# nilspin/VoxelHashing_demo

Hardware: AMD Instinct MI355X
Metric: frames/s TSDF-integrated + raycast Mpix/s, 640×480, 1/2/4/8 MI355X (higher is better)
Workload: dtype f32

## Files before the change

voxelhashing_demo_amd/csrc/vh_api_model.hip:

```cpp

static int sweep_and_release(vh_context *c)
{
    int rc;
    if (c->fp.flags & kFlagOverflow) {
        rc = launch(c, kPhaseGc, gc_sweep_overflow_a_kernel, dim3(256), dim3(256), c->fp, c->dp);
        if (rc == VH_OK) rc = launch(c, kPhaseGc, gc_sweep_overflow_b_kernel, dim3(256), dim3(256), c->fp, c->dp);
    } else {
        rc = launch(c, kPhaseGc, gc_sweep_kernel, dim3(256), dim3(256), c->fp, c->dp);
    }
    if (rc != VH_OK) return rc;
    rc = release_color(c);
    if (rc != VH_OK) return rc;
    rc = launch(c, kPhaseGc, gc_release_kernel, dim3(1024), dim3(256), c->dp);
    if (rc != VH_OK) return rc;
    rc = launch(c, kPhaseGc, gc_finish_kernel, dim3(1), dim3(1), c->dp, c->occupiedCounter);
    if (rc != VH_OK) return rc;
    if (c->profiling) c->times.gc_calls += 1;
    c->params.numOccupiedBlocks = 0;
    VH_HIP(hipGetLastError());
    return VH_OK;
}

extern "C" int vh_delete_blocks(vh_context *c, const int32_t *d_keys, int32_t n)
{
// ... 333 lines not shown
                   : fail(VH_ERR_HIP, "snapshot upload failed; the model was reset to empty", e);
    }
    std::memcpy(c->params.global_transform, h.params.global_transform, sizeof c->fp.T);
    std::memcpy(c->params.inv_global_transform, h.params.inv_global_transform, sizeof c->fp.Tinv);
    std::memcpy(c->fp.T, h.params.global_transform, sizeof c->fp.T);
    std::memcpy(c->fp.Tinv, h.params.inv_global_transform, sizeof c->fp.Tinv);
    std::memcpy(c->fp.proj, h.proj, sizeof h.proj);
    c->params.numOccupiedBlocks = 0;
    c->epochTotal = h.epoch;
    return VH_OK;
}

extern "C" int vh_set_option(vh_context *c, const char *name, int value)
{
    if (c) { DeviceGuard fguard(c->device); const int frc = flush_pending(c); if (frc != VH_OK) return frc; }
    if (!c || !name) return fail(VH_ERR_INVALID_ARGUMENT, "null argument");
    if (std::strcmp(name, "flatten_variant") == 0) {
        if (value != kWalkStridedBallot && value != kWalkIndexed)
            return fail(VH_ERR_INVALID_ARGUMENT, "flatten_variant: 3 (the reference's walk) or 4 (occupancy index)");
        c->flattenVariant = value;
        return VH_OK;
    }
    if (std::strcmp(name, "walk_nt") == 0) {
        c->fp.flags = value ? (c->fp.flags | kFlagWalkNt) : (c->fp.flags & ~kFlagWalkNt);
        return VH_OK;
    }
    if (std::strcmp(name, "walk_reverse") == 0) { c->walkReverse = value != 0; return VH_OK; }
    if (std::strcmp(name, "walk_short") == 0) {
        c->fp.flags = value ? (c->fp.flags | kFlagWalkShort) : (c->fp.flags & ~kFlagWalkShort);
        return VH_OK;
    }
    if (std::strcmp(name, "claim_lead") == 0 && value >= -1) { c->claimLead = value; return VH_OK; }
#ifdef VH_DEBUG_SKIP_ROLES
    if (std::strcmp(name, "debug_skip_roles") == 0 && value >= 0 && value < 32) {
        c->debugSkipRoles = value;
        if (value & 16) c->fp.flags |= kFlagDebugNoProbe; else c->fp.flags &= ~kFlagDebugNoProbe;
        return VH_OK;
    }
#endif
    if (std::strcmp(name, "spin_limit") == 0 && value >= 0) { c->spinLimit = (uint32_t)value; return VH_OK; }
    if (std::strcmp(name, "pipeline_overflow") == 0 && value >= 0 && value <= 2) {
        DeviceGuard g(c->device);
        const int frc = flush_pending(c);
        if (frc != VH_OK) return frc;
        c->pipelineOverflow = value;
        return VH_OK;
    }
    if (std::strcmp(name, "gen_frames_per_launch") == 0 && value >= 1 && value <= kGenBatch) { c->genFramesPerLaunch = value; return VH_OK; }
    if (std::strcmp(name, "pipeline_shards") == 0) {
        if (value < 0 || value > 2) return fail(VH_ERR_INVALID_ARGUMENT, "pipeline_shards: 0, 1 or 2");
        if (value < 2) { DeviceGuard g(c->device); const int frc = flush_pending(c, PendingFrame::kMulti); if (frc != VH_OK) return frc; }
        c->pipelineShards = value;
        return VH_OK;
    }
    if (std::strcmp(name, "pipeline") == 0) {
        c->pipeline = value != 0;
        return VH_OK;
    }
    if (std::strcmp(name, "overflow_list") == 0) {
        if (c->epochTotal != 0 && ((c->fp.flags & kFlagOverflow) != 0u) != (value != 0))
            return fail(VH_ERR_INVALID_ARGUMENT, "overflow_list must be chosen before the first frame");
        if (c->fp.listSize < 2 && value) return fail(VH_ERR_INVALID_ARGUMENT, "attachedLinkedListSize must be at least 2");
        c->fp.flags = value ? (c->fp.flags | kFlagOverflow) : (c->fp.flags & ~kFlagOverflow);
        return VH_OK;
    }
    if (std::strcmp(name, "band_mode") == 0 && (value == VH_BAND_RAY || value == VH_BAND_NORMAL_DDA || value == VH_BAND_RAY_DDA)) {
        c->fp.flags &= ~(kFlagBandDda | kFlagBandRayDda);
// ... 124 lines not shown
```

voxelhashing_demo_amd/csrc/vh_api_shard.hip:

```cpp

static void make_view_frustum(const vh_context *c, const float pose[16], float t_min, float t_max, float f[22])
{
    float inv[16];
    invert4x4(pose, inv);
    std::memcpy(f, inv, 12 * sizeof(float));
    const float r = 7.0f * c->fp.voxelSize;
    const float a[4] = {(0.0f - c->rc_cx) / c->rc_fx, ((float)(c->fp.width - 1) - c->rc_cx) / c->rc_fx,
                        (0.0f - c->rc_cy) / c->rc_fy, ((float)(c->fp.height - 1) - c->rc_cy) / c->rc_fy};
    for (int i = 0; i < 4; ++i) {
        f[12 + i] = a[i];
        f[16 + i] = -(r * sqrtf(1.0f + a[i] * a[i]));
    }
    f[20] = t_min - r;
    f[21] = t_max + r;
}

extern "C" int vh_export_views(vh_context *c, const float *poses, int32_t n_views, float t_min, float t_max,
                               vh_view_record *d_records, int32_t capacity, int32_t *d_counts)
{
    if (!c || !poses || !d_records || !d_counts) return fail(VH_ERR_INVALID_ARGUMENT, "null argument");
    if (n_views < 1 || n_views > VH_MAX_CAMERAS) return fail(VH_ERR_INVALID_ARGUMENT, "1..VH_MAX_CAMERAS views");
    if (capacity < 1) return fail(VH_ERR_INVALID_ARGUMENT, "capacity must be positive");
    if (!(t_max > t_min)) return fail(VH_ERR_INVALID_ARGUMENT, "t_max must exceed t_min");
    if (c->viewBlocks) return fail(VH_ERR_INVALID_ARGUMENT, "a view table has no voxels of its own to export");
// ... 302 lines not shown
        for (int j = 0; j < n; ++j) {
            const int rc = vh_set_pose(c, poses + 16 * (size_t)(b0 + j));
            if (rc != VH_OK) return rc;
            if (!d_depth[b0 + j]) return fail(VH_ERR_INVALID_ARGUMENT, "null depth image");
            std::memcpy(fr.T[j], c->fp.T, sizeof fr.T[j]);
            std::memcpy(fr.Tinv[j], c->fp.Tinv, sizeof fr.Tinv[j]);
            fr.depth[j] = d_depth[b0 + j];
        }
        write_packets_u16_kernel<<<dim3(64, (unsigned)n), 256, 0, c->stream>>>(
            fr, (int32_t)npix, d_packets + packet_frame_stride * (size_t)b0, packet_frame_stride);
    }
    VH_HIP(hipGetLastError());
    return VH_OK;
}

struct MultiBatch {
    const int4 *bins;
    const float *packets;
    int32_t numBins, capacity, binStride, frameStride, numCams;
    size_t packetStride, packetFrameStride;
    bool perBatch;
};

static int launch_multi_pipelined(vh_context *c, const MultiBatch *mb, int b, const GenJob *job)
{
    PendingFrame &pend = c->pend;
    const bool doNew = mb != nullptr, hasOld = pend.kind == PendingFrame::kMulti;
    if (!doNew && !hasOld) return VH_OK;
    int rc;
    if (doNew && (rc = vh_reset_mutexes(c)) != VH_OK) return rc;
    uint32_t *maskOf[2] = {c->dp.compactMask, c->maskBuf2};
    MultiPipeArgs a;
    std::memset(&a, 0, sizeof a);
    PipeRotation r = pipe_rotation(c, a, a, doNew, hasOld);
    a.numEntries = (uint32_t)c->numEntries;
    a.numCams = doNew ? mb->numCams : pend.numCams;
    a.packetStride = doNew ? mb->packetStride : pend.packetStride;
    if (doNew) {
        a.partsPerBin = bin_parts(mb->capacity); a.numBins = (uint32_t)mb->numBins;
        a.claimBlocks = a.numBins * a.partsPerBin;
        a.walkShort = multi_walk_short(c) ? 1u : 0u;
        a.walkIndexed = multi_walk_indexed(c) ? 1u : 0u;
        a.walkBlocks = multi_walk_blocks(c);
        a.capacity = mb->capacity; a.binStride = mb->binStride;
        a.binsNew = mb->bins + (size_t)mb->frameStride * b;
        a.binFrame = mb->perBatch ? b : -1;
        a.packetsNew = mb->packets + mb->packetFrameStride * b;
    }
    a.commitBlocks = hasOld ? (uint32_t)c->commitBlocks : 0u;
    a.integrateBlocks = hasOld ? (uint32_t)c->pipeIntegrateGrid : 0u;
    a.claimSpan = claim_span(c, a.claimBlocks, a.walkBlocks);
    a.claimRatio = claim_ratio(a.claimBlocks, a.claimSpan);
    a.epochOld = pend.epoch;
    a.packetsOld = pend.packets;
    r.dpNew.compactMask = maskOf[r.newParity];
    a.claimOld = r.dpOld.claim; a.candOld = r.dpOld.candidates; a.compactOld = r.dpOld.compact; a.maskOld = maskOf[r.oldParity];
    a.candCapacityOld = r.dpOld.candCapacity;
    const bool sensor = (doNew ? c->packetFormat : pend.packetFormat) == VH_PACKET_U16;
    const bool serial = (c->fp.flags & kFlagOverflow) != 0u;
    const bool gen = job && job->blocks && doNew && sensor && !serial;
    if (gen) a.gen = *job;
    const dim3 grid(a.commitBlocks + a.integrateBlocks + (gen ? a.gen.blocks : 0u) + a.claimBlocks + a.walkBlocks);
    using Yes = std::true_type;
    using No = std::false_type;
    auto go = [&](auto sensorC, auto serialC, auto indexedC, auto genC) {
        return launch(c, kPhaseFramePipelined,
                      frame_multi_pipelined_kernel<decltype(sensorC)::value, decltype(serialC)::value, decltype(indexedC)::value, decltype(genC)::value>,
                      grid, dim3(256), c->fp, r.dpNew, a);
    };
    if (gen) rc = with_bool(a.walkIndexed != 0u, [&](auto i) { return go(Yes{}, No{}, i, Yes{}); });
    else if (a.walkIndexed) rc = with_bool(sensor, [&](auto s) { return go(s, No{}, Yes{}, No{}); });
    else rc = with_bool(sensor, [&](auto s) { return with_bool(serial, [&](auto q) { return go(s, q, No{}, No{}); }); });
    if (rc != VH_OK) return rc;
    pipe_launched(c, r, serial, doNew ? PendingFrame::kMulti : PendingFrame::kNone, hasOld, false, hasOld);
    if (doNew) {
        pend.epoch = c->fp.epoch;
        pend.packets = a.packetsNew;
        pend.packetStride = mb->packetStride;
        pend.numCams = mb->numCams;
        pend.packetFormat = c->packetFormat;
    }
    return VH_OK;
}

static bool multi_can_pipeline(const vh_context *c, int32_t num_bins, int32_t capacity)
{
    return can_pipeline(c, (uint32_t)num_bins * bin_parts(capacity) + (uint32_t)grid_for(c->numEntries, kFlattenThreads * kEntriesPerLaneShort));
}

static bool multi_can_fuse_generation(const vh_context *c, int32_t num_bins, int32_t capacity)
{
    return c->pipelineShards && multi_can_pipeline(c, num_bins, capacity) && !(c->fp.flags & kFlagOverflow) &&
           c->packetFormat == VH_PACKET_U16 && !(c->fp.allocBand > 0.0f) && c->flattenVariant != kWalkIndexed;
}

static bool multi_fusing_pays(const vh_context *c)
{
    return (size_t)c->numEntries * sizeof(VoxelEntry) > ((size_t)60 << 20);
}

static int vh_apply_frames_batch_gen(vh_context *c, int32_t batch, const int32_t *d_bins, int32_t num_bins,
                                     int32_t capacity, int32_t bin_stride, int32_t frame_stride, int32_t num_cams,
                                     const float *d_packets, size_t packet_stride, size_t packet_frame_stride, const GenJob *jobs);

// ... 140 lines not shown
```

voxelhashing_demo_amd/csrc/vh_frame.hip:

```cpp
#pragma once

namespace vh {

__device__ __forceinline__ bool grouped_role(uint32_t r, uint32_t claimBlocks, uint32_t claimSpan, uint32_t claimRatio,
                                             uint32_t claimLead, uint32_t &index)
{
    const uint32_t g = (r >> 3) - claimLead, q = r & 7u;
    uint32_t before = (int32_t)g < 0 ? 0u : (claimBlocks + 7u) >> 3;
    if (g < claimSpan) {
        const unsigned long long phase = (unsigned long long)q << 29;
        before = (uint32_t)(((unsigned long long)g * claimRatio + phase) >> 32);
        const uint32_t after = (uint32_t)(((unsigned long long)(g + 1u) * claimRatio + phase) >> 32);
        if (after != before) { index = 8u * before + q; return true; }
    }
    index = r - 8u * before;
    return false;
}

template <int kKind, class In>
__global__ __launch_bounds__(256) void frame_scan_claim_kernel(const FrameParams fp, const DevPtrs dp, const In in,
                                                               uint32_t numEntries, uint32_t claimBlocks,
                                                               int parity, float *__restrict__ planeOut, uint32_t claimSpan,
                                                               uint32_t claimRatio, uint32_t walkGroups, uint32_t walkReverse,
                                                               uint32_t claimLead)
// ... 146 lines not shown
    kLeanIndexedWaveNt = 8,
    kLeanBuilds = 9
};
struct LeanBuild { uint32_t flags; bool indexed, claimPerWave; };
constexpr LeanBuild lean_build(int kLean)
{
    return {kFlagWalkShort | (kLean % 2 == 0 ? kFlagWalkNt : 0u) | (kLean == kLeanRayDda || kLean == kLeanRayDdaNt ? kFlagBandRayDda : 0u),
            kLean >= kLeanIndexed, kLean >= kLeanIndexedWave};
}

template <bool kSerial>
__device__ __forceinline__ bool pending_live(uint32_t hasOld, const int32_t *counters, int32_t setOld)
{
    if (kSerial) return hasOld != 0u;
    return hasOld && counters[kPipeHeapFree + setOld] >= counters[kPipeWinners + setOld];
}

template <class In, class Depth>
struct PipeKernargs {
    FrameParams fpNew;
    DevPtrs dpNew;
    In inNew;
    FrameParams fpOld;
    DevPtrs dpOld;
    Depth depthOld;
    PipeArgs a;
};
template <class In, class Depth>
struct PipeSignature {
    PipeLeadWords lead;
    PipeKernargs<In, Depth> rest;
};

template <class In, class Depth, int kLean>
__device__ __forceinline__ const PipeKernargs<In, Depth> &role_arguments()
{
    typedef PipeKernargs<In, Depth> K;
    typedef PipeSignature<In, Depth> Signature;
    static_assert(offsetof(Signature, lead) == 0 && offsetof(Signature, rest) == sizeof(PipeLeadWords),
                  "frame_pipelined_kernel(lead, rest): rest lies right behind lead");
    typedef const __attribute__((address_space(4))) char *SegmentBytes;
    typedef const __attribute__((address_space(4))) K *SegmentPtr;
    SegmentPtr p = (SegmentPtr)((SegmentBytes)__builtin_amdgcn_kernarg_segment_ptr() + offsetof(Signature, rest));
    asm volatile("" : "+s"(p));
    const K &k = *(const K *)p;
    constexpr uint32_t leanFlags = lean_build(kLean).flags;
    if (kLean != kLeanNone) {
        __builtin_assume(k.fpNew.flags == leanFlags);
        __builtin_assume(k.fpOld.flags == leanFlags);
    }
    return k;
}

template <class In, class Depth, bool kBand, bool kSerial, int kLean>
__device__ __forceinline__ void frame_pipelined(const PipeLead &l)
{
    typedef PipeKernargs<In, Depth> K;
    constexpr LeanBuild lean = lean_build(kLean);
    const bool walkIndexed = kLean != kLeanNone ? lean.indexed : l.walkIndexed != 0u;
    constexpr bool serial = kSerial;
    const uint32_t b = blockIdx.x;
    uint32_t role, index;
    if (b < l.commitBlocks) { role = 0; index = b; }
    else if (walkIndexed) {
        const uint32_t r = b - l.commitBlocks;
        if (r < l.walkBlocks) { role = 3; index = r; }
        else if (r < l.walkBlocks + l.integrateBlocks) { role = 1; index = r - l.walkBlocks; }
        else { role = 2; index = r - l.walkBlocks - l.integrateBlocks; }
    }
    else if (b < l.commitBlocks + l.integrateBlocks) { role = 1; index = b - l.commitBlocks; }
    else {
        const bool claims = grouped_role(b - l.commitBlocks - l.integrateBlocks, l.claimBlocks, l.claimSpan, l.claimRatio, l.claimLead, index);
        role = claims ? 2u : 3u;
        if (claims && index >= l.claimBlocks) return;
    }
#ifdef VH_DEBUG_SKIP_ROLES
    if (l.skipRoles & (1u << role)) {
        const K &k = role_arguments<In, Depth, kLean>();
// ... 150 lines not shown
```

voxelhashing_demo_amd/csrc/vh_shard.hip:

```cpp
#pragma once

namespace vh {

constexpr int kBinFrameMarks = 0x40000000;

__device__ __forceinline__ void claim_bin_slice(const FrameParams &fp, const DevPtrs &dp,
                                                const int4 *__restrict__ bins, int32_t capacity, int32_t binStride,
                                                uint32_t binIndex, uint32_t part, uint32_t parts, int candCounter,
                                                const Pending &pend = kNoPending, int frame = -1)
{
    const int4 *bin = bins + (size_t)binIndex * binStride;
    const int4 head = bin[0];
    int n = head.x;
    const bool frameMarks = frame >= 0 && (head.w & kBinFrameMarks) != 0;
    const int room = frameMarks ? capacity - 3 : capacity - 1;
    int lo = 0, hiMark = 0;
    if (frameMarks) {
        const int4 c0 = bin[capacity - 2], c1 = bin[capacity - 1];
        const int cnt[8] = {c0.x, c0.y, c0.z, c0.w, c1.x, c1.y, c1.z, c1.w};
        n = 0;
#pragma unroll
        for (int f = 0; f < 8; ++f) {
            if (f == frame) lo = n;
            n += cnt[f];
            if (f == frame) hiMark = n;
        }
    }
    if (n > room) {
        if (part == 0 && threadIdx.x == 0) atomicAdd(dp.counters + kBinOverflow, 1);
        n = room;
    }
    if (frameMarks) {
        lo = min(lo, n);
        n = min(hiMark, n);
    } else if (frame >= 0 && head.w != 0) {
        const int per = head.w & 0xff, marks = (head.w >> 8) & 0xff, g = frame / per;
        const int m0 = min(head.y, n), m1 = min(head.z, n);
        lo = g == 0 ? 0 : g == 1 ? m0 : m1;
        n = g < marks ? (g == 0 ? m0 : m1) : n;
        if (g > 2) lo = n;
    }
#ifdef VH_DEBUG_SKIP_ROLES
    if (fp.flags & kFlagDebugNoProbe) n = min(n, lo + ((n - lo) >> 5));
#endif
    for (int i = lo + (int)part * 256 + (int)threadIdx.x; i < n; i += (int)parts * 256) {
        const int4 k = bin[1 + i];
        uint32_t rank = (uint32_t)k.w;
        if (frame >= 0) {
            if ((rank >> kRankCameraShift) != (uint32_t)frame) continue;
            rank = (binIndex << kRankCameraShift) | (rank & ((1u << kRankCameraShift) - 1u));
        }
        const uint32_t h = hash_block(k.x, k.y, k.z, fp.numBuckets);
        if (h < fp.bucketLo || h >= fp.bucketHi) continue;
        probe_and_claim(fp, dp, k.x, k.y, k.z, h, rank, candCounter, pend);
    }
}

__global__ __launch_bounds__(256) void claim_bins_kernel(const FrameParams fp, const DevPtrs dp,
                                                         const int4 *__restrict__ bins, int32_t capacity,
                                                         int32_t binStride)
{
    claim_bin_slice(fp, dp, bins, capacity, binStride, blockIdx.y, blockIdx.x, gridDim.x, kCandCount);
}

__device__ __forceinline__ uint32_t camera_mask(const FrameParams &fp, const int *pos, int32_t numCams,
                                                const float *__restrict__ packets, size_t packetStride)
{
    uint32_t seen = 0;
    for (int c = 0; c < numCams; ++c) {
        const float *pk = packets + packetStride * c;
        if (block_in_frustum(fp, pk, pk + 16, pos[0], pos[1], pos[2])) seen |= 1u << c;
    }
    return seen;
}

template <int kN = kEntriesPerLane>
__device__ __forceinline__ void flatten_multi_tile(const FrameParams &fp, const DevPtrs &dp, uint32_t numEntries,
                                                   uint32_t tileIndex, int32_t numCams,
                                                   const float *__restrict__ packets, size_t packetStride,
                                                   int counter, const Pending &pend = kNoPending)
{
    const uint32_t tile = tileIndex * (kFlattenThreads * kN);
    int32_t ptrs[kN];
    walk_load_tile(fp, dp, numEntries, tileIndex, ptrs);
    uint32_t seen[kN];
    int myCount = 0;
#pragma unroll
    for (int j = 0; j < kN; ++j) {
        seen[j] = 0;
        if (ptrs[j] == VH_FREE_BLOCK) continue;
        const uint32_t e = tile + j * kFlattenThreads + threadIdx.x;
        const VoxelEntry ent = dp.table[e];
        if (pend.claim && pend.live) {
            const uint32_t b = e / fp.bucketSize;
            const unsigned long long w = pend.claim[b];
            if (claim_epoch(w) == pend.epoch && claim_f(w) == e - b * fp.bucketSize) continue;
        }
        seen[j] = camera_mask(fp, ent.pos, numCams, packets, packetStride);
        myCount += seen[j] != 0u;
    }
    int slot = reserve_compact_slots(dp, counter, myCount);
    if (slot < 0) return;
#pragma unroll
    for (int j = 0; j < kN; ++j) {
        if (seen[j] == 0u) continue;
        dp.compact[slot] = dp.table[tile + j * kFlattenThreads + threadIdx.x];
        dp.compactMask[slot] = seen[j];
        ++slot;
    }
}

struct IndexSinkMulti {
    const FrameParams &fp;
    int32_t numCams;
    const float *__restrict__ packets;
    size_t packetStride;
    int counterIndex;
    __device__ __forceinline__ uint32_t judge(const VoxelEntry &e) const { return camera_mask(fp, e.pos, numCams, packets, packetStride); }
    __device__ __forceinline__ int counter() const { return counterIndex; }
    __device__ __forceinline__ void emit(const DevPtrs &dp, uint32_t pos, const VoxelEntry &e, uint32_t seen) const
    {
        dp.compact[pos] = e;
        dp.compactMask[pos] = seen;
    }
};

__global__ __launch_bounds__(kFlattenThreads) void flatten_multi_kernel(const FrameParams fp, const DevPtrs dp,
                                                                        uint32_t numEntries, int32_t numCams,
                                                                        const float *__restrict__ packets,
                                                                        size_t packetStride)
{
    flatten_multi_tile(fp, dp, numEntries, blockIdx.x, numCams, packets, packetStride, kCompactCount);
}

template <bool kSensor>
__device__ __forceinline__ auto packet_depth(const float *pk)
{
    if constexpr (kSensor) return DepthSensor{reinterpret_cast<const uint16_t *>(pk + kPacketHeaderU16), pk[32], pk[33], pk[34], pk[35]};
    else return DepthPlane{pk + kPacketHeader, 1};
}

template <bool kSensor>
// ... 79 lines not shown
                    dp.compactMask[slot] = seen;
                }
            }
        }
        __syncthreads();
        if (inserted && newMask != 0u)
            integrate_block_multi<kSensor>(fp, dp, newEntry, newMask, numCams, packets, packetStride);
        __syncthreads();
    }
    close_commit_fused(dp.counters, workers, parity, scanCount, 0, demanded);
}

#ifndef VH_FUSED_GEN_GROUPS
#define VH_FUSED_GEN_GROUPS 6
#endif
#ifndef VH_FUSED_GEN_PRIO
#define VH_FUSED_GEN_PRIO 3
#endif
constexpr int kFusedGenGroups = VH_FUSED_GEN_GROUPS;
struct GenJob {
    uint32_t blocks;
    int32_t numShards, capacity, binStride;
    int4 *bins;
    float *packet;
    const uint16_t *depth;
    uint32_t rankBase;
    float T[16], Tinv[16], k[9], unit;
    int4 *clearBins;
    int32_t clearStride;
    int32_t frame, batch;
};


struct MultiPipeArgs {
    uint32_t claimBlocks, walkBlocks, commitBlocks, integrateBlocks;
    uint32_t partsPerBin, numBins, numEntries;
    int32_t capacity, binStride, numCams;
    int32_t binFrame;
    int32_t doneTag;
    uint32_t spinLimit;
    int32_t setNew, setOld, setClear;
    uint32_t hasNew, hasOld;
    uint32_t walkShort;
    uint32_t walkIndexed;
    uint32_t claimSpan, claimRatio;
    uint32_t epochOld;
    const int4 *binsNew;
    const float *packetsNew, *packetsOld;
    size_t packetStride;
    unsigned long long *claimOld;
    int4 *candOld;
    VoxelEntry *compactOld;
    uint32_t *maskOld;
    uint32_t candCapacityOld;
    GenJob gen;
};

template <bool kSensor, bool kSerial, bool kIndexed = false, bool kGen = false>
__global__ __launch_bounds__(256) void frame_multi_pipelined_kernel(const FrameParams fp, const DevPtrs dp, const MultiPipeArgs a)
{
    if (!a.hasOld && blockIdx.x == 0u && threadIdx.x == 0) dp.counters[kPipeHeapFree + a.setNew] = dp.counters[kHeapCounter] + 1;
    if constexpr (kGen) {
        const uint32_t g0 = a.commitBlocks + a.integrateBlocks;
        if (blockIdx.x >= g0 && blockIdx.x < g0 + a.gen.blocks) {
            const uint32_t g = blockIdx.x - g0;
            if (VH_FUSED_GEN_PRIO) __builtin_amdgcn_s_setprio(VH_FUSED_GEN_PRIO);
            FrameParams fg = fp;
#pragma unroll
            for (int i = 0; i < 16; ++i) { fg.T[i] = a.gen.T[i]; fg.Tinv[i] = a.gen.Tinv[i]; }
            SensorImage in;
            in.depth = a.gen.depth;
#pragma unroll
            for (int i = 0; i < 9; ++i) in.k[i] = a.gen.k[i];
            in.unit = a.gen.unit;
            float *pk = a.gen.packet;
            if (g == 0 && threadIdx.x < kPacketHeaderU16) {
                const int t = threadIdx.x;
                pk[t] = t < 16 ? a.gen.T[t] : t < 32 ? a.gen.Tinv[t - 16] : t == 32 ? a.gen.k[6] : t == 33 ? a.gen.k[7] : t == 34 ? a.gen.k[8] : a.gen.unit;
            }
            if (g == 0 && a.gen.clearBins && (int)threadIdx.x < a.gen.numShards) {
                int4 *nb = a.gen.clearBins + (size_t)threadIdx.x * a.gen.clearStride;
                nb[0] = make_int4(0, 0, 0, kBinFrameMarks | a.gen.batch);
                nb[a.gen.capacity - 2] = make_int4(0, 0, 0, 0);
                nb[a.gen.capacity - 1] = make_int4(0, 0, 0, 0);
            }
#pragma unroll
            for (int j = 0; j < kFusedGenGroups; ++j) {
                const int idx = ((int)g * kFusedGenGroups + j) * 256 + (int)threadIdx.x;
                if (idx < fp.width * fp.height) reinterpret_cast<uint16_t *>(pk + kPacketHeaderU16)[idx] = in.depth[idx];
            }
            generate_keys_groups<SensorImage, 256, kFusedGenGroups>(fg, in, a.gen.numShards, a.gen.bins, a.gen.capacity - 2, a.gen.binStride, nullptr,
                                                                    a.gen.rankBase, g * (uint32_t)kFusedGenGroups, a.gen.frame);
            return;
        }
    }
    const uint32_t genBlocks = kGen ? a.gen.blocks : 0u;
    int32_t *counters = dp.counters;
    const int demandedOld = a.hasOld ? counters[kPipeCand + a.setOld] : 0;
    const int candOld = min(demandedOld, (int)a.candCapacityOld);
    constexpr bool serial = kSerial;
    const bool live = serial ? a.hasOld != 0u : a.hasOld && counters[kPipeHeapFree + a.setOld] >= counters[kPipeWinners + a.setOld];
    const uint32_t b = blockIdx.x;
    if (b >= a.commitBlocks + a.integrateBlocks + genBlocks) {
        if (!a.hasNew) return;
        if (serial && a.hasOld) {
            if (!wait_commit_done(counters, a.doneTag, a.spinLimit)) return;
        }
        const Pending pend{a.hasOld && !serial ? a.claimOld : nullptr, a.candOld, a.epochOld, live, serial ? -1 : kPipeWinners + a.setNew};
        const uint32_t r = b - a.commitBlocks - a.integrateBlocks - genBlocks;
        uint32_t before = a.claimBlocks, after = a.claimBlocks;
        if constexpr (kIndexed) {
            if (r < a.walkBlocks) {
                flatten_index_tile_to(fp, dp, r, IndexSinkMulti{fp, a.numCams, a.packetsNew, a.packetStride, kPipeScan + a.setNew}, pend);
                return;
            }
            before = r - a.walkBlocks; after = before + 1u;
        }
        else { if (r < a.claimSpan) { before = __umulhi(r, a.claimRatio); after = __umulhi(r + 1u, a.claimRatio); } }
        if (after != before) {
            __builtin_amdgcn_s_setprio(3);
            claim_bin_slice(fp, dp, a.binsNew, a.capacity, a.binStride, before / a.partsPerBin, before % a.partsPerBin, a.partsPerBin,
                            kPipeCand + a.setNew, pend, a.binFrame);
        } else {
            if (a.walkShort) flatten_multi_tile<kEntriesPerLaneShort>(fp, dp, a.numEntries, r - before, a.numCams, a.packetsNew, a.packetStride, kPipeScan + a.setNew, pend);
            else flatten_multi_tile(fp, dp, a.numEntries, r - before, a.numCams, a.packetsNew, a.packetStride, kPipeScan + a.setNew, pend);
        }
        return;
    }
    if (!a.hasOld) return;
    const int scanOld = counters[kPipeScan + a.setOld];
    if (b >= a.commitBlocks) {
        for (int k = (int)(b - a.commitBlocks); k < scanOld; k += (int)a.integrateBlocks)
            integrate_block_multi<kSensor>(fp, dp, a.compactOld[k], a.maskOld[k], a.numCams, a.packetsOld, a.packetStride);
        return;
    }
    __shared__ VoxelEntry newEntry;
    __shared__ uint32_t newMask;
    __shared__ int inserted;
    const int workers = max(1, min(candOld, (int)a.commitBlocks));
    if ((int)b >= workers) return;
    for (int i = (int)b; i < candOld; i += (int)a.commitBlocks) {
        if (threadIdx.x == 0) {
            inserted = 0;
            newMask = 0u;
            const int4 k = a.candOld[i];
            if (live) {
                VoxelEntry e;
                inserted = commit_candidate(fp, dp, k, e, (uint32_t)i, false, a.epochOld, a.claimOld) ? 1 : 0;
                if (inserted) {
                    const uint32_t seen = camera_mask(fp, e.pos, a.numCams, a.packetsOld, a.packetStride);
                    newEntry = e;
                    newMask = seen;
                    if (seen != 0u) {
                        const int slot = scanOld + atomicAdd(counters + kPipeNew + a.setOld, 1);
                        a.compactOld[slot] = e;
                        a.maskOld[slot] = seen;
                    }
                    if (a.hasNew && !serial) {
                        const uint32_t next = camera_mask(fp, e.pos, a.numCams, a.packetsNew, a.packetStride);
                        if (next != 0u) {
                            const int slot = atomicAdd(counters + kPipeScan + a.setNew, 1);
                            dp.compact[slot] = e;
                            dp.compactMask[slot] = next;
                        }
                    }
                }
            } else {
                const uint32_t local = hash_block(k.x, k.y, k.z, fp.numBuckets) - fp.bucketLo;
                const unsigned long long w = a.claimOld[local];
                if (claim_epoch(w) == a.epochOld && claim_slot(w) == (uint32_t)i) atomicAdd(counters + kHeapExhausted, 1);
            }
        }
        __syncthreads();
        if (inserted && newMask != 0u)
            integrate_block_multi<kSensor>(fp, dp, newEntry, newMask, a.numCams, a.packetsOld, a.packetStride);
        __syncthreads();
    }
    if (threadIdx.x == 0) {
        __threadfence();
        const int ticket = atomicAdd(counters + kCommitTicket, 1);
        if (ticket == workers - 1) {
            counters[kCompactCount] = scanOld + atomicAdd(counters + kPipeNew + a.setOld, 0);
            counters[kLastCandidates] = demandedOld;
            clear_pipe_set(counters, a.setClear);
            if (!a.hasNew) clear_pipe_set(counters, a.setNew);
            counters[kPipeHeapFree + a.setNew] = atomicAdd(counters + kHeapCounter, 0) + 1;
            counters[kCommitTicket] = 0;
            if (serial) {
                __threadfence();
                __hip_atomic_store(counters + kPipeCommitDone, a.doneTag, __ATOMIC_RELAXED, __HIP_MEMORY_SCOPE_AGENT);
            }
        }
    }
}

struct SensorFrames {
    float T[kGenBatch][16];
    float Tinv[kGenBatch][16];
    const uint16_t *depth[kGenBatch];
    float k6, k7, k8, unit;
};

__global__ __launch_bounds__(256) void write_packets_u16_kernel(const SensorFrames fr, int32_t numPixels,
                                                                float *__restrict__ packets, size_t packetFrameStride)
{
    const int b = blockIdx.y;
    float *pk = packets + packetFrameStride * b;
    if (blockIdx.x == 0 && threadIdx.x < kPacketHeaderU16) {
        const int t = threadIdx.x;
        pk[t] = t < 16 ? fr.T[b][t] : t < 32 ? fr.Tinv[b][t - 16] : t == 32 ? fr.k6 : t == 33 ? fr.k7 : t == 34 ? fr.k8 : fr.unit;
    }
    const uint32_t *src = reinterpret_cast<const uint32_t *>(fr.depth[b]);
    uint32_t *dst = reinterpret_cast<uint32_t *>(pk + kPacketHeaderU16);
    const int words = numPixels / 2;
    for (int i = blockIdx.x * 256 + threadIdx.x; i < words; i += gridDim.x * 256) dst[i] = src[i];
}

__global__ void bin_mark_kernel(int4 *bins, int32_t numShards, int32_t binStride, int32_t g, int32_t framesPerLaunch, int32_t marks)
{
    const int i = blockIdx.x * blockDim.x + threadIdx.x;
    if (i >= numShards) return;
    int4 *head = bins + (size_t)i * binStride;
    const int count = head->x;
    if (g == 0) head->y = count; else head->z = count;
    head->w = framesPerLaunch | (marks << 8);
}

// ... 20 lines not shown
```

Baseline: 64750.

## Pack multi-pipeline role dispatch fields into a 64-byte lead kernarg

Restructures the multi-camera pipelined frame kernel so the role-dispatch fields (block counts, claim ratio, walk settings, table pointer, flags) sit in a 64-byte lead struct loaded as one scalar load. The remaining FrameParams, DevPtrs and args are read lazily from the kernarg segment only by the roles that need them. The walk role issues its table loads before touching the bulk arguments. This is meant to cut scalar-load latency and SGPR pressure at kernel entry. It adds layout static_asserts and a debug role-skip mask, and it depends on fragile kernarg-offset assumptions.

```diff
diff --git a/voxelhashing_demo_amd/csrc/vh_api_model.hip b/voxelhashing_demo_amd/csrc/vh_api_model.hip
--- a/voxelhashing_demo_amd/csrc/vh_api_model.hip
+++ b/voxelhashing_demo_amd/csrc/vh_api_model.hip
@@ -389,7 +389,7 @@
     }
     if (std::strcmp(name, "claim_lead") == 0 && value >= -1) { c->claimLead = value; return VH_OK; }
 #ifdef VH_DEBUG_SKIP_ROLES
-    if (std::strcmp(name, "debug_skip_roles") == 0 && value >= 0 && value < 32) {
+    if (std::strcmp(name, "debug_skip_roles") == 0 && value >= 0 && value < 64) {
         c->debugSkipRoles = value;
         if (value & 16) c->fp.flags |= kFlagDebugNoProbe; else c->fp.flags &= ~kFlagDebugNoProbe;
         return VH_OK;
diff --git a/voxelhashing_demo_amd/csrc/vh_api_shard.hip b/voxelhashing_demo_amd/csrc/vh_api_shard.hip
--- a/voxelhashing_demo_amd/csrc/vh_api_shard.hip
+++ b/voxelhashing_demo_amd/csrc/vh_api_shard.hip
@@ -358,25 +358,29 @@
     uint32_t *maskOf[2] = {c->dp.compactMask, c->maskBuf2};
     MultiPipeArgs a;
     std::memset(&a, 0, sizeof a);
-    PipeRotation r = pipe_rotation(c, a, a, doNew, hasOld);
-    a.numEntries = (uint32_t)c->numEntries;
+    MultiPipeLead l{};
+    PipeRotation r = pipe_rotation(c, a, l, doNew, hasOld);
+    l.table = r.dpNew.table;
+    l.flags = c->fp.flags;
+    l.numEntries = (uint32_t)c->numEntries;
     a.numCams = doNew ? mb->numCams : pend.numCams;
     a.packetStride = doNew ? mb->packetStride : pend.packetStride;
+    bool walkIndexed = false;
     if (doNew) {
-        a.partsPerBin = bin_parts(mb->capacity); a.numBins = (uint32_t)mb->numBins;
-        a.claimBlocks = a.numBins * a.partsPerBin;
-        a.walkShort = multi_walk_short(c) ? 1u : 0u;
-        a.walkIndexed = multi_walk_indexed(c) ? 1u : 0u;
-        a.walkBlocks = multi_walk_blocks(c);
+        a.partsPerBin = bin_parts(mb->capacity);
+        l.claimBlocks = (uint32_t)mb->numBins * a.partsPerBin;
+        l.walkShort = multi_walk_short(c) ? 1u : 0u;
+        walkIndexed = multi_walk_indexed(c);
+        l.walkBlocks = multi_walk_blocks(c);
         a.capacity = mb->capacity; a.binStride = mb->binStride;
         a.binsNew = mb->bins + (size_t)mb->frameStride * b;
         a.binFrame = mb->perBatch ? b : -1;
         a.packetsNew = mb->packets + mb->packetFrameStride * b;
     }
-    a.commitBlocks = hasOld ? (uint32_t)c->commitBlocks : 0u;
-    a.integrateBlocks = hasOld ? (uint32_t)c->pipeIntegrateGrid : 0u;
-    a.claimSpan = claim_span(c, a.claimBlocks, a.walkBlocks);
-    a.claimRatio = claim_ratio(a.claimBlocks, a.claimSpan);
+    l.commitBlocks = hasOld ? (uint32_t)c->commitBlocks : 0u;
+    l.integrateBlocks = hasOld ? (uint32_t)c->pipeIntegrateGrid : 0u;
+    l.claimSpan = claim_span(c, l.claimBlocks, l.walkBlocks);
+    l.claimRatio = claim_ratio(l.claimBlocks, l.claimSpan);
     a.epochOld = pend.epoch;
     a.packetsOld = pend.packets;
     r.dpNew.compactMask = maskOf[r.newParity];
@@ -385,17 +389,21 @@
     const bool sensor = (doNew ? c->packetFormat : pend.packetFormat) == VH_PACKET_U16;
     const bool serial = (c->fp.flags & kFlagOverflow) != 0u;
     const bool gen = job && job->blocks && doNew && sensor && !serial;
-    if (gen) a.gen = *job;
-    const dim3 grid(a.commitBlocks + a.integrateBlocks + (gen ? a.gen.blocks : 0u) + a.claimBlocks + a.walkBlocks);
+    if (gen) { a.gen = *job; l.genBlocks = job->blocks; }
+#ifdef VH_DEBUG_SKIP_ROLES
+    l.skipRoles = (uint32_t)c->debugSkipRoles;
+#endif
+    const dim3 grid(l.commitBlocks + l.integrateBlocks + l.genBlocks + l.claimBlocks + l.walkBlocks);
+    const MultiPipeSignature sig{__builtin_bit_cast(PipeLeadWords, l), {c->fp, r.dpNew, a}};
     using Yes = std::true_type;
     using No = std::false_type;
     auto go = [&](auto sensorC, auto serialC, auto indexedC, auto genC) {
         return launch(c, kPhaseFramePipelined,
                       frame_multi_pipelined_kernel<decltype(sensorC)::value, decltype(serialC)::value, decltype(indexedC)::value, decltype(genC)::value>,
-                      grid, dim3(256), c->fp, r.dpNew, a);
+                      grid, dim3(256), sig.lead, sig.rest);
     };
-    if (gen) rc = with_bool(a.walkIndexed != 0u, [&](auto i) { return go(Yes{}, No{}, i, Yes{}); });
-    else if (a.walkIndexed) rc = with_bool(sensor, [&](auto s) { return go(s, No{}, Yes{}, No{}); });
+    if (gen) rc = with_bool(walkIndexed, [&](auto i) { return go(Yes{}, No{}, i, Yes{}); });
+    else if (walkIndexed) rc = with_bool(sensor, [&](auto s) { return go(s, No{}, Yes{}, No{}); });
     else rc = with_bool(sensor, [&](auto s) { return with_bool(serial, [&](auto q) { return go(s, q, No{}, No{}); }); });
     if (rc != VH_OK) return rc;
     pipe_launched(c, r, serial, doNew ? PendingFrame::kMulti : PendingFrame::kNone, hasOld, false, hasOld);
diff --git a/voxelhashing_demo_amd/csrc/vh_frame.hip b/voxelhashing_demo_amd/csrc/vh_frame.hip
--- a/voxelhashing_demo_amd/csrc/vh_frame.hip
+++ b/voxelhashing_demo_amd/csrc/vh_frame.hip
@@ -202,18 +202,23 @@
     PipeKernargs<In, Depth> rest;
 };
 
-template <class In, class Depth, int kLean>
-__device__ __forceinline__ const PipeKernargs<In, Depth> &role_arguments()
-{
-    typedef PipeKernargs<In, Depth> K;
-    typedef PipeSignature<In, Depth> Signature;
-    static_assert(offsetof(Signature, lead) == 0 && offsetof(Signature, rest) == sizeof(PipeLeadWords),
-                  "frame_pipelined_kernel(lead, rest): rest lies right behind lead");
+template <class Signature>
+__device__ __forceinline__ auto signature_rest() -> const decltype(Signature::rest) &
+{
+    typedef decltype(Signature::rest) K;
+    static_assert(std::is_same<decltype(Signature::lead), PipeLeadWords>::value && offsetof(Signature, lead) == 0 &&
+                  offsetof(Signature, rest) == sizeof(PipeLeadWords), "kernel(lead, rest): rest lies right behind the 64 bytes of lead");
     typedef const __attribute__((address_space(4))) char *SegmentBytes;
     typedef const __attribute__((address_space(4))) K *SegmentPtr;
     SegmentPtr p = (SegmentPtr)((SegmentBytes)__builtin_amdgcn_kernarg_segment_ptr() + offsetof(Signature, rest));
     asm volatile("" : "+s"(p));
-    const K &k = *(const K *)p;
+    return *(const K *)p;
+}
+template <class In, class Depth, int kLean>
+__device__ __forceinline__ const PipeKernargs<In, Depth> &role_arguments()
+{
+    typedef PipeKernargs<In, Depth> K;
+    const K &k = signature_rest<PipeSignature<In, Depth>>();
     constexpr uint32_t leanFlags = lean_build(kLean).flags;
     if (kLean != kLeanNone) {
         __builtin_assume(k.fpNew.flags == leanFlags);
diff --git a/voxelhashing_demo_amd/csrc/vh_shard.hip b/voxelhashing_demo_amd/csrc/vh_shard.hip
--- a/voxelhashing_demo_amd/csrc/vh_shard.hip
+++ b/voxelhashing_demo_amd/csrc/vh_shard.hip
@@ -4,10 +4,12 @@
 
 constexpr int kBinFrameMarks = 0x40000000;
 
-__device__ __forceinline__ void claim_bin_slice(const FrameParams &fp, const DevPtrs &dp,
-                                                const int4 *__restrict__ bins, int32_t capacity, int32_t binStride,
-                                                uint32_t binIndex, uint32_t part, uint32_t parts, int candCounter,
-                                                const Pending &pend = kNoPending, int frame = -1)
+struct BinSlice {
+    const int4 *bin;
+    int lo, n;
+};
+__device__ __forceinline__ BinSlice claim_bin_range(const FrameParams &fp, const DevPtrs &dp, const int4 *__restrict__ bins, int32_t capacity,
+                                                    int32_t binStride, uint32_t binIndex, uint32_t part, int frame)
 {
     const int4 *bin = bins + (size_t)binIndex * binStride;
     const int4 head = bin[0];
@@ -43,8 +45,13 @@
 #ifdef VH_DEBUG_SKIP_ROLES
     if (fp.flags & kFlagDebugNoProbe) n = min(n, lo + ((n - lo) >> 5));
 #endif
-    for (int i = lo + (int)part * 256 + (int)threadIdx.x; i < n; i += (int)parts * 256) {
-        const int4 k = bin[1 + i];
+    return {bin, lo, n};
+}
+__device__ __forceinline__ void claim_bin_records(const FrameParams &fp, const DevPtrs &dp, const BinSlice &s, uint32_t binIndex, uint32_t part,
+                                                  uint32_t parts, int candCounter, const Pending &pend, int frame)
+{
+    for (int i = s.lo + (int)part * 256 + (int)threadIdx.x; i < s.n; i += (int)parts * 256) {
+        const int4 k = s.bin[1 + i];
         uint32_t rank = (uint32_t)k.w;
         if (frame >= 0) {
             if ((rank >> kRankCameraShift) != (uint32_t)frame) continue;
@@ -55,6 +62,14 @@
         probe_and_claim(fp, dp, k.x, k.y, k.z, h, rank, candCounter, pend);
     }
 }
+__device__ __forceinline__ void claim_bin_slice(const FrameParams &fp, const DevPtrs &dp,
+                                                const int4 *__restrict__ bins, int32_t capacity, int32_t binStride,
+                                                uint32_t binIndex, uint32_t part, uint32_t parts, int candCounter,
+                                                const Pending &pend = kNoPending, int frame = -1)
+{
+    const BinSlice s = claim_bin_range(fp, dp, bins, capacity, binStride, binIndex, part, frame);
+    claim_bin_records(fp, dp, s, binIndex, part, parts, candCounter, pend, frame);
+}
 
 __global__ __launch_bounds__(256) void claim_bins_kernel(const FrameParams fp, const DevPtrs dp,
                                                          const int4 *__restrict__ bins, int32_t capacity,
@@ -74,15 +89,13 @@
     return seen;
 }
 
-template <int kN = kEntriesPerLane>
-__device__ __forceinline__ void flatten_multi_tile(const FrameParams &fp, const DevPtrs &dp, uint32_t numEntries,
-                                                   uint32_t tileIndex, int32_t numCams,
-                                                   const float *__restrict__ packets, size_t packetStride,
-                                                   int counter, const Pending &pend = kNoPending)
+template <int kN>
+__device__ __forceinline__ void flatten_multi_process(const FrameParams &fp, const DevPtrs &dp, uint32_t tileIndex,
+                                                      const int32_t (&ptrs)[kN], int32_t numCams,
+                                                      const float *__restrict__ packets, size_t packetStride,
+                                                      int counter, const Pending &pend = kNoPending)
 {
     const uint32_t tile = tileIndex * (kFlattenThreads * kN);
-    int32_t ptrs[kN];
-    walk_load_tile(fp, dp, numEntries, tileIndex, ptrs);
     uint32_t seen[kN];
     int myCount = 0;
 #pragma unroll
@@ -108,6 +121,16 @@
         dp.compactMask[slot] = seen[j];
         ++slot;
     }
+}
+template <int kN = kEntriesPerLane>
+__device__ __forceinline__ void flatten_multi_tile(const FrameParams &fp, const DevPtrs &dp, uint32_t numEntries,
+                                                   uint32_t tileIndex, int32_t numCams,
+                                                   const float *__restrict__ packets, size_t packetStride,
+                                                   int counter, const Pending &pend = kNoPending)
+{
+    int32_t ptrs[kN];
+    walk_load_tile(fp, dp, numEntries, tileIndex, ptrs);
+    flatten_multi_process(fp, dp, tileIndex, ptrs, numCams, packets, packetStride, counter, pend);
 }
 
 struct IndexSinkMulti {
@@ -253,18 +276,26 @@
 };
 
 
+struct MultiPipeLead {
+    uint32_t commitBlocks, integrateBlocks, genBlocks, claimBlocks, walkBlocks;
+    uint32_t claimSpan, claimRatio;
+    uint32_t hasNew, hasOld;
+    uint32_t numEntries;
+    uint32_t walkShort;
+    uint32_t flags;
+    uint32_t skipRoles;
+    uint32_t unused;
+    const VoxelEntry *table;
+};
+static_assert(sizeof(MultiPipeLead) == sizeof(PipeLeadWords), "MultiPipeLead is the one 64-byte scalar load at the head of the arguments");
+
 struct MultiPipeArgs {
-    uint32_t claimBlocks, walkBlocks, commitBlocks, integrateBlocks;
-    uint32_t partsPerBin, numBins, numEntries;
+    uint32_t partsPerBin;
     int32_t capacity, binStride, numCams;
     int32_t binFrame;
     int32_t doneTag;
     uint32_t spinLimit;
     int32_t setNew, setOld, setClear;
-    uint32_t hasNew, hasOld;
-    uint32_t walkShort;
-    uint32_t walkIndexed;
-    uint32_t claimSpan, claimRatio;
     uint32_t epochOld;
     const int4 *binsNew;
     const float *packetsNew, *packetsOld;
@@ -276,98 +307,161 @@
     uint32_t candCapacityOld;
     GenJob gen;
 };
-
-template <bool kSensor, bool kSerial, bool kIndexed = false, bool kGen = false>
-__global__ __launch_bounds__(256) void frame_multi_pipelined_kernel(const FrameParams fp, const DevPtrs dp, const MultiPipeArgs a)
-{
-    if (!a.hasOld && blockIdx.x == 0u && threadIdx.x == 0) dp.counters[kPipeHeapFree + a.setNew] = dp.counters[kHeapCounter] + 1;
+struct MultiPipeKernargs {
+    FrameParams fp;
+    DevPtrs dp;
+    MultiPipeArgs a;
+};
+struct MultiPipeSignature {
+    PipeLeadWords lead;
+    MultiPipeKernargs rest;
+};
+
+template <bool kSensor, bool kSerial, bool kIndexed, bool kGen>
+__device__ __forceinline__ void frame_multi_pipelined(const MultiPipeLead &l)
+{
+    typedef MultiPipeKernargs K;
+    constexpr bool serial = kSerial;
+    const uint32_t b = blockIdx.x;
+    const uint32_t deferred = l.commitBlocks + l.integrateBlocks, genBlocks = kGen ? l.genBlocks : 0u;
+    uint32_t role, index;
+    if (b < l.commitBlocks) { role = 0; index = b; }
+    else if (b < deferred) { role = 1; index = b - l.commitBlocks; }
+    else if (b < deferred + genBlocks) { role = 5; index = b - deferred; }
+    else {
+        const uint32_t r = b - deferred - genBlocks;
+        if constexpr (kIndexed) {
+            if (r < l.walkBlocks) { role = 3; index = r; }
+            else { role = 2; index = r - l.walkBlocks; }
+        } else {
+            uint32_t before = l.claimBlocks, after = l.claimBlocks;
+            if (r < l.claimSpan) { before = __umulhi(r, l.claimRatio); after = __umulhi(r + 1u, l.claimRatio); }
+            if (after != before) { role = 2; index = before; }
+            else { role = 3; index = r - before; }
+        }
+    }
+#ifdef VH_DEBUG_SKIP_ROLES
+    if (l.skipRoles & (1u << role)) {
+        const K &k = signature_rest<MultiPipeSignature>();
+        if (role == 0u && b == 0u && threadIdx.x == 0 && l.hasOld) {
+            clear_pipe_set(k.dp.counters, k.a.setClear);
+            if (!l.hasNew) clear_pipe_set(k.dp.counters, k.a.setNew);
+        }
+        if (!l.hasOld && role == 2u && index == 0u && threadIdx.x == 0)
+            k.dp.counters[kPipeHeapFree + k.a.setNew] = k.dp.counters[kHeapCounter] + 1;
+        return;
+    }
+#endif
     if constexpr (kGen) {
-        const uint32_t g0 = a.commitBlocks + a.integrateBlocks;
-        if (blockIdx.x >= g0 && blockIdx.x < g0 + a.gen.blocks) {
-            const uint32_t g = blockIdx.x - g0;
+        if (role == 5u) {
+            const K &k = signature_rest<MultiPipeSignature>();
+            const GenJob &gen = k.a.gen;
+            const uint32_t g = index;
             if (VH_FUSED_GEN_PRIO) __builtin_amdgcn_s_setprio(VH_FUSED_GEN_PRIO);
-            FrameParams fg = fp;
+            FrameParams fg = k.fp;
 #pragma unroll
-            for (int i = 0; i < 16; ++i) { fg.T[i] = a.gen.T[i]; fg.Tinv[i] = a.gen.Tinv[i]; }
+            for (int i = 0; i < 16; ++i) { fg.T[i] = gen.T[i]; fg.Tinv[i] = gen.Tinv[i]; }
             SensorImage in;
-            in.depth = a.gen.depth;
+            in.depth = gen.depth;
 #pragma unroll
-            for (int i = 0; i < 9; ++i) in.k[i] = a.gen.k[i];
-            in.unit = a.gen.unit;
-            float *pk = a.gen.packet;
+            for (int i = 0; i < 9; ++i) in.k[i] = gen.k[i];
+            in.unit = gen.unit;
+            float *pk = gen.packet;
             if (g == 0 && threadIdx.x < kPacketHeaderU16) {
                 const int t = threadIdx.x;
-                pk[t] = t < 16 ? a.gen.T[t] : t < 32 ? a.gen.Tinv[t - 16] : t == 32 ? a.gen.k[6] : t == 33 ? a.gen.k[7] : t == 34 ? a.gen.k[8] : a.gen.unit;
-            }
-            if (g == 0 && a.gen.clearBins && (int)threadIdx.x < a.gen.numShards) {
-                int4 *nb = a.gen.clearBins + (size_t)threadIdx.x * a.gen.clearStride;
-                nb[0] = make_int4(0, 0, 0, kBinFrameMarks | a.gen.batch);
-                nb[a.gen.capacity - 2] = make_int4(0, 0, 0, 0);
-                nb[a.gen.capacity - 1] = make_int4(0, 0, 0, 0);
+                pk[t] = t < 16 ? gen.T[t] : t < 32 ? gen.Tinv[t - 16] : t == 32 ? gen.k[6] : t == 33 ? gen.k[7] : t == 34 ? gen.k[8] : gen.unit;
+            }
+            if (g == 0 && gen.clearBins && (int)threadIdx.x < gen.numShards) {
+                int4 *nb = gen.clearBins + (size_t)threadIdx.x * gen.clearStride;
+                nb[0] = make_int4(0, 0, 0, kBinFrameMarks | gen.batch);
+                nb[gen.capacity - 2] = make_int4(0, 0, 0, 0);
+                nb[gen.capacity - 1] = make_int4(0, 0, 0, 0);
             }
 #pragma unroll
             for (int j = 0; j < kFusedGenGroups; ++j) {
                 const int idx = ((int)g * kFusedGenGroups + j) * 256 + (int)threadIdx.x;
-                if (idx < fp.width * fp.height) reinterpret_cast<uint16_t *>(pk + kPacketHeaderU16)[idx] = in.depth[idx];
-            }
-            generate_keys_groups<SensorImage, 256, kFusedGenGroups>(fg, in, a.gen.numShards, a.gen.bins, a.gen.capacity - 2, a.gen.binStride, nullptr,
-                                                                    a.gen.rankBase, g * (uint32_t)kFusedGenGroups, a.gen.frame);
+                if (idx < fg.width * fg.height) reinterpret_cast<uint16_t *>(pk + kPacketHeaderU16)[idx] = in.depth[idx];
+            }
+            generate_keys_groups<SensorImage, 256, kFusedGenGroups>(fg, in, gen.numShards, gen.bins, gen.capacity - 2, gen.binStride, nullptr,
+                                                                    gen.rankBase, g * (uint32_t)kFusedGenGroups, gen.frame);
             return;
         }
     }
-    const uint32_t genBlocks = kGen ? a.gen.blocks : 0u;
+    if (role >= 2u) {
+        if (!l.hasNew) return;
+        if (serial && l.hasOld) {
+            const K &k = signature_rest<MultiPipeSignature>();
+            if (!wait_commit_done(k.dp.counters, k.a.doneTag, k.a.spinLimit)) return;
+        }
+        const auto pending = [&](const K &k) {
+            return Pending{l.hasOld && !serial ? k.a.claimOld : nullptr, k.a.candOld, k.a.epochOld,
+                           pending_live<serial>(l.hasOld, k.dp.counters, k.a.setOld), serial ? -1 : kPipeWinners + k.a.setNew};
+        };
+        if constexpr (!kIndexed) {
+            if (role == 3u) {
+                typedef const __attribute__((address_space(1))) VoxelEntry *GlobalTable;
+                FrameParams loadFp{};
+                DevPtrs loadDp{};
+                loadFp.flags = l.flags;
+                loadDp.table = (VoxelEntry *)(GlobalTable)(uintptr_t)l.table;
+                const auto walk = [&](auto &ptrs) {
+                    walk_load_tile(loadFp, loadDp, l.numEntries, index, ptrs);
+                    if (!walk_wave_live(ptrs)) return;
+                    const K &k = signature_rest<MultiPipeSignature>();
+                    flatten_multi_process(k.fp, k.dp, index, ptrs, k.a.numCams, k.a.packetsNew, k.a.packetStride, kPipeScan + k.a.setNew, pending(k));
+                };
+                if (l.walkShort) {
+                    int32_t ptrs[kEntriesPerLaneShort];
+                    walk(ptrs);
+                } else {
+                    int32_t ptrs[kEntriesPerLane];
+                    walk(ptrs);
+                }
+                return;
+            }
+        }
+        const K &k = signature_rest<MultiPipeSignature>();
+        if (role == 3u) {
+            flatten_index_tile_to(k.fp, k.dp, index, IndexSinkMulti{k.fp, k.a.numCams, k.a.packetsNew, k.a.packetStride, kPipeScan + k.a.setNew}, pending(k));
+            return;
+        }
+        __builtin_amdgcn_s_setprio(3);
+        const uint32_t binIndex = index / k.a.partsPerBin, part = index % k.a.partsPerBin;
+        const BinSlice s = claim_bin_range(k.fp, k.dp, k.a.binsNew, k.a.capacity, k.a.binStride, binIndex, part, k.a.binFrame);
+        const Pending pend = pending(k);
+        if (!l.hasOld && index == 0u && threadIdx.x == 0) k.dp.counters[kPipeHeapFree + k.a.setNew] = k.dp.counters[kHeapCounter] + 1;
+        claim_bin_records(k.fp, k.dp, s, binIndex, part, k.a.partsPerBin, kPipeCand + k.a.setNew, pend, k.a.binFrame);
+        return;
+    }
+    if (!l.hasOld) return;
+    const K &k = signature_rest<MultiPipeSignature>();
+    const FrameParams &fp = k.fp;
+    const DevPtrs &dp = k.dp;
+    const MultiPipeArgs &a = k.a;
     int32_t *counters = dp.counters;
-    const int demandedOld = a.hasOld ? counters[kPipeCand + a.setOld] : 0;
+    if (role == 1u) {
+        const int scanOld = counters[kPipeScan + a.setOld];
+        for (int i = (int)index; i < scanOld; i += (int)l.integrateBlocks)
+            integrate_block_multi<kSensor>(fp, dp, a.compactOld[i], a.maskOld[i], a.numCams, a.packetsOld, a.packetStride);
+        return;
+    }
+    const int demandedOld = counters[kPipeCand + a.setOld];
+    const int scanOld = counters[kPipeScan + a.setOld];
+    const bool live = pending_live<serial>(l.hasOld, counters, a.setOld);
     const int candOld = min(demandedOld, (int)a.candCapacityOld);
-    constexpr bool serial = kSerial;
-    const bool live = serial ? a.hasOld != 0u : a.hasOld && counters[kPipeHeapFree + a.setOld] >= counters[kPipeWinners + a.setOld];
-    const uint32_t b = blockIdx.x;
-    if (b >= a.commitBlocks + a.integrateBlocks + genBlocks) {
-        if (!a.hasNew) return;
-        if (serial && a.hasOld) {
-            if (!wait_commit_done(counters, a.doneTag, a.spinLimit)) return;
-        }
-        const Pending pend{a.hasOld && !serial ? a.claimOld : nullptr, a.candOld, a.epochOld, live, serial ? -1 : kPipeWinners + a.setNew};
-        const uint32_t r = b - a.commitBlocks - a.integrateBlocks - genBlocks;
-        uint32_t before = a.claimBlocks, after = a.claimBlocks;
-        if constexpr (kIndexed) {
-            if (r < a.walkBlocks) {
-                flatten_index_tile_to(fp, dp, r, IndexSinkMulti{fp, a.numCams, a.packetsNew, a.packetStride, kPipeScan + a.setNew}, pend);
-                return;
-            }
-            before = r - a.walkBlocks; after = before + 1u;
-        }
-        else { if (r < a.claimSpan) { before = __umulhi(r, a.claimRatio); after = __umulhi(r + 1u, a.claimRatio); } }
-        if (after != before) {
-            __builtin_amdgcn_s_setprio(3);
-            claim_bin_slice(fp, dp, a.binsNew, a.capacity, a.binStride, before / a.partsPerBin, before % a.partsPerBin, a.partsPerBin,
-                            kPipeCand + a.setNew, pend, a.binFrame);
-        } else {
-            if (a.walkShort) flatten_multi_tile<kEntriesPerLaneShort>(fp, dp, a.numEntries, r - before, a.numCams, a.packetsNew, a.packetStride, kPipeScan + a.setNew, pend);
-            else flatten_multi_tile(fp, dp, a.numEntries, r - before, a.numCams, a.packetsNew, a.packetStride, kPipeScan + a.setNew, pend);
-        }
-        return;
-    }
-    if (!a.hasOld) return;
-    const int scanOld = counters[kPipeScan + a.setOld];
-    if (b >= a.commitBlocks) {
-        for (int k = (int)(b - a.commitBlocks); k < scanOld; k += (int)a.integrateBlocks)
-            integrate_block_multi<kSensor>(fp, dp, a.compactOld[k], a.maskOld[k], a.numCams, a.packetsOld, a.packetStride);
-        return;
-    }
     __shared__ VoxelEntry newEntry;
     __shared__ uint32_t newMask;
     __shared__ int inserted;
-    const int workers = max(1, min(candOld, (int)a.commitBlocks));
-    if ((int)b >= workers) return;
-    for (int i = (int)b; i < candOld; i += (int)a.commitBlocks) {
+    const int workers = max(1, min(candOld, (int)l.commitBlocks));
+    if ((int)index >= workers) return;
+    for (int i = (int)index; i < candOld; i += (int)l.commitBlocks) {
         if (threadIdx.x == 0) {
             inserted = 0;
             newMask = 0u;
-            const int4 k = a.candOld[i];
+            const int4 key = a.candOld[i];
             if (live) {
                 VoxelEntry e;
-                inserted = commit_candidate(fp, dp, k, e, (uint32_t)i, false, a.epochOld, a.claimOld) ? 1 : 0;
+                inserted = commit_candidate(fp, dp, key, e, (uint32_t)i, false, a.epochOld, a.claimOld) ? 1 : 0;
                 if (inserted) {
                     const uint32_t seen = camera_mask(fp, e.pos, a.numCams, a.packetsOld, a.packetStride);
                     newEntry = e;
@@ -377,7 +471,7 @@
                         a.compactOld[slot] = e;
                         a.maskOld[slot] = seen;
                     }
-                    if (a.hasNew && !serial) {
+                    if (l.hasNew && !serial) {
                         const uint32_t next = camera_mask(fp, e.pos, a.numCams, a.packetsNew, a.packetStride);
                         if (next != 0u) {
                             const int slot = atomicAdd(counters + kPipeScan + a.setNew, 1);
@@ -387,7 +481,7 @@
                     }
                 }
             } else {
-                const uint32_t local = hash_block(k.x, k.y, k.z, fp.numBuckets) - fp.bucketLo;
+                const uint32_t local = hash_block(key.x, key.y, key.z, fp.numBuckets) - fp.bucketLo;
                 const unsigned long long w = a.claimOld[local];
                 if (claim_epoch(w) == a.epochOld && claim_slot(w) == (uint32_t)i) atomicAdd(counters + kHeapExhausted, 1);
             }
@@ -404,7 +498,7 @@
             counters[kCompactCount] = scanOld + atomicAdd(counters + kPipeNew + a.setOld, 0);
             counters[kLastCandidates] = demandedOld;
             clear_pipe_set(counters, a.setClear);
-            if (!a.hasNew) clear_pipe_set(counters, a.setNew);
+            if (!l.hasNew) clear_pipe_set(counters, a.setNew);
             counters[kPipeHeapFree + a.setNew] = atomicAdd(counters + kHeapCounter, 0) + 1;
             counters[kCommitTicket] = 0;
             if (serial) {
@@ -414,6 +508,18 @@
         }
     }
 }
+
+#pragma clang diagnostic push
+#pragma clang diagnostic ignored "-Wpsabi"
+template <bool kSensor, bool kSerial, bool kIndexed = false, bool kGen = false>
+__global__ __launch_bounds__(256) void frame_multi_pipelined_kernel(const PipeLeadWords lead, const MultiPipeKernargs)
+{
+    static_assert(std::is_same<decltype(MultiPipeSignature::lead), PipeLeadWords>::value &&
+                  std::is_same<decltype(MultiPipeSignature::rest), MultiPipeKernargs>::value, "keep MultiPipeSignature in step");
+    const MultiPipeLead l = __builtin_bit_cast(MultiPipeLead, lead);
+    frame_multi_pipelined<kSensor, kSerial, kIndexed, kGen>(l);
+}
+#pragma clang diagnostic pop
 
 struct SensorFrames {
     float T[kGenBatch][16];
```

New measurement: 64940 (median of 6 runs). Within noise of the previous version (+0.3%).
